# EnVision-Research/Uni-Renderer

Measured on AMD Instinct MI355X. Metric: denoise-steps/sec (dual-UNet, 512^2 bs=4), higher is better.
Workload: dtype f16; 1 GPU; inverse-rendering denoise step: AttributeEncoderModel + UNet2DConditionModel + AttributeDecoderModel forward (SD-1.x size, 1.74 G params, random init), 512x512 image = 64x64 latent, 28-channel attribute latent, 77x768 prompt embedding, batch 4 per GPU; per_gpu_batch=4, global_batch=4, parallelism=dp1, residual_stream=(hi, lo) pairs (parity <= 1e-3, DESIGN.md section 5)

## Files before the change

### include/ur_kernels.h

```cpp
#ifndef UR_KERNELS_H
#define UR_KERNELS_H

#include <stdint.h>

#ifdef __cplusplus
extern "C" {
#endif

#define UR_ABI_VERSION 13

#define UR_E_BADARG (-1001)
#define UR_E_UNSUPPORTED (-1002)

#define UR_DT_F16 0
#define UR_DT_BF16 1
#define UR_DT_F32 2

#define UR_ACT_NONE 0
#define UR_ACT_SILU 1
#define UR_ACT_GEGLU 2

#define UR_TILE_AUTO 0
#define UR_TILE_128x128 1
#define UR_TILE_128x64 2
#define UR_TILE_64x64 3
#define UR_TILE_128x128_S3 4
#define UR_TILE_128x64_S2 5
#define UR_TILE_64x64_S4 6
#define UR_TILE_64x64_S2 7
#define UR_TILE_256x128 8
#define UR_TILE_128x320 9
#define UR_TILE_128x256 10
#define UR_TILE_256x256 11
#define UR_TILE_64x64_R 12
#define UR_TILE_128x64_R 13
#define UR_TILE_128x128_R 14
#define UR_TILE_128x320_R 15
#define UR_TILE_256x128_R 16
#define UR_TILE_64x64_W1 17
#define UR_TILE_128x64_W2 18
#define UR_TILE_64x64_W1_S3 19
#define UR_TILE_64x128_W2 20
// ... 59 lines not shown
    int32_t c0, c1;
    int32_t B, Hin, Win, Hout, Wout;
    int32_t taps, stride, ups;
    int32_t M, N, K;
    int32_t n_store;
    int32_t ld_rowadd, rows_per_b;
    int32_t act;
    float out_scale;
    int32_t zbatch, splitk;
    int32_t zx_div;
    int32_t tile;
    int32_t dtype;
    const void* res_lo;
    void* out_lo;
    int32_t cblock;
    const void* t0;
    const void* t1;
    int64_t ldt0, ldt1, zt0, zt1;
    int32_t ct0, ct1;
    int32_t pad;
    void* out_vt;
    int64_t ldvt, vt_bstride, zvt;
    int32_t vt_n0, vt_rows;
    int32_t zero_page_bytes;
} ur_igemm_desc;

int ur_igemm(const ur_igemm_desc* d, void* stream);

int ur_igemm_uses_dxs(const ur_igemm_desc* d);

int ur_igemm_splitk_gn(const ur_igemm_desc* d, const float* gamma, const float* beta, int64_t zgn, float eps, int groups,
                       int silu, void* stream);

int ur_has_wsconv(void);
int ur_has_pp(void);

int64_t ur_igemm_partial_floats(const ur_igemm_desc* d);

int ur_groupnorm_stats(const void* x0, const void* x1, const void* x0_lo, const void* x1_lo, int c0, int c1, int B,
                       int rows, int groups, int nchunks, float* partial, int dtype, void* stream);
int ur_groupnorm_apply(const void* x0, const void* x1, const void* x0_lo, const void* x1_lo, int c0, int c1, int B,
                       int rows, int groups, int nstat, int nchunks, const float* partial, const float* gamma,
                       const float* beta, float eps, int silu, int bper, int pstride, void* out, int dtype,
                       void* stream);

#define UR_GN_TWO_SWEEP 2
int ur_groupnorm_fused(const void* x0, const void* x1, const void* x0_lo, const void* x1_lo, int c0, int c1, int B,
                       int rows, int groups, const float* gamma, const float* beta, float eps, int silu, int bper,
                       int pstride, void* out, int dtype, void* stream);

int ur_layernorm(const void* x, const void* x_lo, const float* gamma, const float* beta, float eps, int rows, int C,
                 int rows_per_set, int pstride, void* out, int dtype, void* stream);

typedef struct ur_attn_desc {
    const void* q;
    const void* k;
    const void* vt;
    void* o;
    const void* zero_page;
    int64_t ldq, ldk, ldvt, ldo;
    int64_t vt_bstride;
    int64_t q_hstride, k_hstride;
    int32_t q_off, k_off;
    int32_t B, H, Tq, Tk, d;
    float scale;
    int32_t dtype;
// ... 229 lines not shown
```

### uni_renderer_amd/_experiments.py

```python
from __future__ import annotations

import os

KNOWN = {
    "tchain": "row-local chain kernels at the 320-channel level (fused.py)",
    "qkv_one_launch": "q | k | v as one GEMM with a transposed value output (fused.py)",
    "ctxkv_one_launch": "prompt K | V^T of a phase as one GEMM (fused.py)",
    "vt_first": "V^T projection issued before the q | k projection (only without qkv_one_launch)",
    "exchange_early": "exchange GEMMs right behind the kernel that produced their skip (fused.py)",
    "ctx3_early": "up-phase time / prompt projections issued before phase 1 (fused.py)",
    "fold_shortcut": "resnet conv_shortcut as the 1x1 K tail of conv2 (ops.py)",
    "multi_transpose": "batched weight transposes of the backward (backward.py)",
    "batch_wt": "all W^T of a network in one launch group (backward.py)",
    "fused_gradnorm": "clipping norm collected where the gradients are written (backward.py)",
    "wgrad": "weight gradients on ur_wgrad instead of transposed-operand GEMMs (backward.py)",
    "wgrad_table": "measured (tile, slices) table of ur_wgrad (backward.py)",
    "wgrad_defer": "weight gradients deferred to the end of a network's backward and grouped (backward.py)",
    "norm_defer": "gamma / beta gradient sums deferred to the same barriers (backward.py)",
    "heads_multi": "split / merge heads of several tensors in one launch (backward.py)",
    "flash_backward": "flash attention backward instead of the materialised-P path (backward.py)",
    "forward_lse": "the forward attention hands its row log-sum-exp to the backward (backward.py)",
    "batch_casts": "fp32 -> bf16 parameter casts of a network in one launch group (train_step.py)",
    "gn_resident": "one-launch GroupNorm keeps small strips in registers: one memory round trip (ops.py, csrc/norm.hip)",
    "head_major_qk": "the chain kernels write q / k of the d = 40 attention as [sample][head][token][40] images (fused.py)",
    "splitk_gn": "GroupNorm as the split-K second pass (0.07 ms slower: profiles/r04_splitk_gn_ab.txt)",
    "colsum_one_launch": "column sums with an in-launch ticket instead of two launches (slower)",
    "fused_colsum": "bias gradient sums inside the dx GEMM launch (slower)",
    "side_stream": "=1|2|3: independent launches on a sibling graph branch (0.5 ms slower: DESIGN.md)",
    "wsconv": "weight-streaming conv kernel where K >= wsconv_min_k (needs `make WSCONV=1`; slower in the step)",
    "wsconv_min_k": "", "wsconv_waves": "", "zero_page_bytes": "", "conv_cblock": "", "gn_stat_kb": "", "gn_apply_kb": "",
    "gn_apply_max": "", "gn_fused_max_rows": "", "gn_bwd_fused_max_rows": "", "wgrad_tile": "", "wgrad_splits": "",
    "flash_direct_min_d": "", "tchain_min_rows": "", "gn_resident_max_rows": "",
}

RETIRED = {
    "UR_ATTN_BWD_TRN", "UR_BATCH_CASTS", "UR_BATCH_WT", "UR_COLSUM_ONE_LAUNCH", "UR_CONV_CBLOCK", "UR_CTX3_EARLY",
    "UR_CTXKV_ONE_LAUNCH", "UR_EXCHANGE_EARLY", "UR_FLASH_BACKWARD", "UR_FLASH_DIRECT_MIN_D", "UR_FLASH_M32", "UR_FOLD_SHORTCUT",
    "UR_FORWARD_LSE", "UR_FUSED_COLSUM", "UR_FUSED_GRADNORM", "UR_GNF_XCD", "UR_GN_APPLY_KB", "UR_GN_APPLY_MAX",
    "UR_GN_BWD_FUSED_MAX_ROWS", "UR_GN_FUSED_MAX_ROWS", "UR_GN_STAT_KB", "UR_HEADS_MULTI", "UR_MULTI_TRANSPOSE", "UR_NORM_DEFER",
    "UR_NORM_XCD", "UR_QKV_ONE_LAUNCH", "UR_SIDE_STREAM", "UR_SPLITK_GN", "UR_TCHAIN", "UR_TCHAIN_FF", "UR_TCHAIN_PRE",
    "UR_TCHAIN_Q", "UR_TRANSPOSE_MAX", "UR_VT_FIRST", "UR_WGRAD", "UR_WGRAD_DEFER", "UR_WGRAD_SPLITS", "UR_WGRAD_TABLE",
    "UR_WGRAD_TILE", "UR_WSCONV", "UR_WSCONV_MIN_K", "UR_WSCONV_WAVES", "UR_ZERO_PAGE_BYTES",
}

_parsed = None


def _load():
    global _parsed
    if _parsed is None:
        stale = sorted(k for k in os.environ if k in RETIRED)
        if stale:
            raise ValueError(f"retired environment variable(s) {', '.join(stale)}: no longer read -- use UR_EXPERIMENT=... "
                             f"(uni_renderer_amd/_experiments.py lists the entries)")
        d = {}
        for item in os.environ.get("UR_EXPERIMENT", "").replace(";", ",").split(","):
            item = item.strip()
# ... 23 lines not shown
```

### uni_renderer_amd/_lib.py

```python
from __future__ import annotations

import ctypes as C
import os

import torch

_HERE = os.path.dirname(os.path.abspath(__file__))
LIB_PATH = os.environ.get("UR_LIB_PATH", os.path.join(_HERE, "liburhip.so"))
ABI_VERSION = 13

i32, i64, f32, vp = C.c_int32, C.c_int64, C.c_float, C.c_void_p


class IGemmDesc(C.Structure):

    _fields_ = [
        ("x0", vp), ("x1", vp), ("w", vp), ("bias", vp), ("rowadd", vp), ("res", vp), ("out", vp),
        ("partial", vp), ("zero_page", vp),
        ("ldx0", i64), ("ldx1", i64), ("ldw", i64), ("ldres", i64), ("ldc", i64),
        ("zx", i64), ("zw", i64), ("zout", i64), ("zx1", i64), ("zbias", i64), ("zrow", i64), ("zres", i64),
        ("ldp", i64),
        ("c0", i32), ("c1", i32),
        ("B", i32), ("Hin", i32), ("Win", i32), ("Hout", i32), ("Wout", i32),
        ("taps", i32), ("stride", i32), ("ups", i32),
        ("M", i32), ("N", i32), ("K", i32),
        ("n_store", i32), ("ld_rowadd", i32), ("rows_per_b", i32),
        ("act", i32), ("out_scale", f32),
        ("zbatch", i32), ("splitk", i32), ("zx_div", i32), ("tile", i32), ("dtype", i32),
        ("res_lo", vp), ("out_lo", vp),
        ("cblock", i32),
        ("t0", vp), ("t1", vp), ("ldt0", i64), ("ldt1", i64), ("zt0", i64), ("zt1", i64), ("ct0", i32), ("ct1", i32),
        ("pad", i32),
        ("out_vt", vp), ("ldvt", i64), ("vt_bstride", i64), ("zvt", i64), ("vt_n0", i32), ("vt_rows", i32),
        ("zero_page_bytes", i32),
    ]


class AttnDesc(C.Structure):

    _fields_ = [
        ("q", vp), ("k", vp), ("vt", vp), ("o", vp), ("zero_page", vp),
        ("ldq", i64), ("ldk", i64), ("ldvt", i64), ("ldo", i64), ("vt_bstride", i64),
# ... 3 lines not shown
        ("scale", f32), ("dtype", i32),
        ("lse", vp),
    ]


class AttnBwdDesc(C.Structure):

    _fields_ = [
        ("q", vp), ("k", vp), ("v", vp), ("o", vp), ("dout", vp), ("qt", vp), ("kt", vp), ("dot", vp),
        ("ldq", i64), ("ldk", i64), ("ldv", i64), ("ldo", i64), ("lddo", i64), ("ldqt", i64), ("ldkt", i64), ("lddot", i64),
        ("stats", vp), ("dq", vp), ("dk", vp), ("dv", vp),
        ("lddq", i64), ("lddk", i64), ("lddv", i64),
        ("part", vp),
        ("B", i32), ("H", i32), ("d", i32), ("Tq", i32), ("Tk", i32), ("Tk_rows", i32), ("has_lse", i32),
        ("scale", f32), ("dtype", i32),
    ]


class TChainDesc(C.Structure):

    _fields_ = [
        ("a0", vp), ("res", vp), ("res_lo", vp), ("blk", vp), ("blk_lo", vp), ("y_out", vp), ("y_out_lo", vp),
        ("out", vp), ("out_lo", vp), ("out2", vp), ("out3", vp), ("wstream", vp), ("consts", vp),
        ("z_wstream", i64), ("z_consts", i64),
        ("M", i32), ("zbatch", i32), ("mode", i32), ("dtype", i32), ("channels", i32),
        ("rows_per_b", i32), ("ld_vt", i32), ("qk_heads", i32),
        ("eps", f32),
        ("profile", vp),
    ]


SYMBOLS = {
    "ur_igemm": (C.c_int, [C.POINTER(IGemmDesc), vp]),
    "ur_igemm_partial_floats": (C.c_int64, [C.POINTER(IGemmDesc)]),
    "ur_groupnorm_stats": (C.c_int, [vp, vp, vp, vp, C.c_int, C.c_int, C.c_int, C.c_int, C.c_int, C.c_int, vp, C.c_int, vp]),
    "ur_groupnorm_apply": (C.c_int, [vp, vp, vp, vp, C.c_int, C.c_int, C.c_int, C.c_int, C.c_int, C.c_int, C.c_int, vp, vp,
                                     vp, C.c_float, C.c_int, C.c_int, C.c_int, vp, C.c_int, vp]),
    "ur_groupnorm_fused": (C.c_int, [vp, vp, vp, vp, C.c_int, C.c_int, C.c_int, C.c_int, C.c_int, vp, vp, C.c_float,
                                     C.c_int, C.c_int, C.c_int, vp, C.c_int, vp]),
    "ur_layernorm": (C.c_int, [vp, vp, vp, vp, C.c_float, C.c_int, C.c_int, C.c_int, C.c_int, vp, C.c_int, vp]),
    "ur_attention": (C.c_int, [C.POINTER(AttnDesc), vp]),
    "ur_add": (C.c_int, [vp, vp, C.c_float, vp, C.c_int64, C.c_int, vp]),
    "ur_add_hilo": (C.c_int, [vp, vp, vp, vp, C.c_float, vp, vp, C.c_int64, C.c_int, vp]),
    "ur_add_hilo_multi": (C.c_int, [vp, C.c_int, C.c_int, vp]),
    "ur_sizeof_add_item": (C.c_int, []),
    "ur_timestep_embedding": (C.c_int, [vp, C.c_int, C.c_int, C.c_int, C.c_int, C.c_float, vp, C.c_int, vp]),
    "ur_resize_nearest": (C.c_int, [vp, vp, C.c_int, C.c_int, C.c_int, C.c_int, C.c_int, C.c_int, C.c_int, vp]),
    "ur_nchw_to_nhwc": (C.c_int, [vp, C.c_int, C.c_int, C.c_int, C.c_int, C.c_int, vp, C.c_int, C.c_int, vp]),
    "ur_nhwc_to_nchw": (C.c_int, [vp, C.c_int, C.c_int, C.c_int, C.c_int, C.c_int, vp, C.c_int, vp]),
    "ur_ddim_update": (C.c_int, [vp, C.c_int, C.c_int, vp, C.c_int64, C.c_int, C.c_int, C.c_int, vp, vp, C.c_int, vp,
                                 C.c_int, C.c_int, C.c_float, C.c_int, C.c_int, vp]),
    "ur_sampler_advance": (C.c_int, [vp, vp, C.c_int, vp, C.c_int, vp]),
    "ur_select_step_rows": (C.c_int, [vp, vp, vp, C.c_int, vp, C.c_int, vp]),
    "ur_prefetch": (C.c_int, [vp, C.c_int64, C.c_int, vp]),
    "ur_pack_conv_weight": (C.c_int, [vp, vp, C.c_int, C.c_int, C.c_int, C.c_int, vp]),
    "ur_unpack_conv_weight_grad": (C.c_int, [vp, C.c_int64, vp, C.c_int, C.c_int, C.c_int, C.c_int, vp]),
    "ur_unpack_conv_weight_grad_blocks": (C.c_int, [C.c_int, C.c_int]),
    "ur_unpack_conv_weight_grad_sumsq": (C.c_int, [vp, C.c_int64, vp, C.c_int, C.c_int, C.c_int, vp, C.c_int, vp]),
    "ur_unipc_update": (C.c_int, [vp, C.c_int, C.c_int, vp, C.c_int64, C.c_int, C.c_int, C.c_int, vp, vp, C.c_int, vp, vp,
                                  vp, C.c_int, C.c_int, C.c_float, C.c_int, C.c_int, vp]),
    "ur_transpose2d": (C.c_int, [vp, C.c_int64, C.c_int64, vp, C.c_int64, C.c_int64, C.c_int, C.c_int, C.c_int, C.c_int, vp]),
    "ur_im2col3x3_t": (C.c_int, [vp, C.c_int, C.c_int, C.c_int, C.c_int, C.c_int, vp, C.c_int64, C.c_int, vp]),
    "ur_colsum_workspace_floats": (C.c_int64, [C.c_int, C.c_int, C.c_int]),
    "ur_colsum": (C.c_int, [vp, C.c_int64, C.c_int, C.c_int, C.c_int, vp, vp, C.c_int, vp]),
    "ur_colsum_counters": (C.c_int, [C.c_int, C.c_int, C.c_int]),
    "ur_colsum_fused": (C.c_int, [vp, C.c_int64, C.c_int, C.c_int, C.c_int, vp, vp, vp, C.c_int, vp]),
# ... 115 lines not shown
```

### uni_renderer_amd/csrc/igemm.hip

```cpp
#include <cstdlib>

#include "igemm_epi.h"

namespace ur {

template <typename T, int BM, int BN, int WM, int WN, int NSTAGE, bool CONV, int MF, int NL>
__global__ void __launch_bounds__((WM * WN + NL) * 64) igemm_kernel(const ur_igemm_desc p) {
    typedef typename Vec8<T>::type vec8;
    constexpr int NWC = WM * WN;
    constexpr int NW = NL > 0 ? NL : NWC;
    static_assert(NL == 0 || NSTAGE > 0, "loader waves use the LDS-DMA ring");
    constexpr int MREP = BM / WM / 16;
    constexpr int NREP = BN / WN / 16;
    static_assert(MF == 16 || MF == 32, "MFMA shape");
    static_assert(MF == 32 || NREP == 4, "a wave spans 64 output columns (epilogue layout)");
    static_assert(MF == 16 || ((BM / WM) % 32 == 0 && (BN / WN) % 32 == 0), "32x32 MFMA: wave tile in multiples of 32");
    constexpr int MI = BM / WM / 32, NI = BN / WN / 32;
    constexpr int XT_BYTES = BM * 128;
    constexpr int WT_BYTES = BN * 128;
    constexpr int STAGE = XT_BYTES + WT_BYTES;
    constexpr bool REGSTAGE = NSTAGE < 0;
    constexpr int XI = (BM / 8 + NW - 1) / NW;
    constexpr int WI = (BN / 8 + NW - 1) / NW;
    static_assert(NSTAGE <= 2 || ((BM / 8) % NW == 0 && (BN / 8) % NW == 0), "counted vmcnt needs uniform loads per wave");
// ... 706 lines not shown
        case UR_TILE_256x256_M32: return launch_cfg<T, 256, 256, 4, 4, 2, 32>(d, s, reduce);
        case UR_TILE_256x128_M32: return launch_cfg<T, 256, 128, 4, 2, 2, 32>(d, s, reduce);
        case UR_TILE_128x256_M32: return launch_cfg<T, 128, 256, 2, 4, 2, 32>(d, s, reduce);
        case UR_TILE_128x320_L2: return launch_cfg<T, 128, 320, 2, 5, 2, 16, 2>(d, s, reduce);
        case UR_TILE_128x320_L4: return launch_cfg<T, 128, 320, 2, 5, 2, 16, 4>(d, s, reduce);
        case UR_TILE_128x128_L2: return launch_cfg<T, 128, 128, 2, 2, 2, 16, 2>(d, s, reduce);
        case UR_TILE_128x128_S3_L2: return launch_cfg<T, 128, 128, 2, 2, 3, 16, 2>(d, s, reduce);
        case UR_TILE_128x64_L1: return launch_cfg<T, 128, 64, 4, 1, 2, 16, 1>(d, s, reduce);
        case UR_TILE_128x64_S3_L2: return launch_cfg<T, 128, 64, 4, 1, 3, 16, 2>(d, s, reduce);
        case UR_TILE_64x64_S3_L1: return launch_cfg<T, 64, 64, 4, 1, 3, 16, 1>(d, s, reduce);
        case UR_TILE_256x128_L2: return launch_cfg<T, 256, 128, 4, 2, 2, 16, 2>(d, s, reduce);
        case UR_TILE_256x256_L0: return UR_E_UNSUPPORTED;
        case UR_TILE_128x256_L2: return launch_cfg<T, 128, 256, 2, 4, 2, 16, 2>(d, s, reduce);
        case UR_TILE_128x256_S3: return launch_cfg<T, 128, 256, 2, 4, 3>(d, s, reduce);
        case UR_TILE_128x320_W8_M32: return launch_cfg<T, 128, 320, 4, 2, 2, 32>(d, s, reduce);
        case UR_TILE_256x320_W16_M32: return launch_cfg<T, 256, 320, 8, 2, 2, 32>(d, s, reduce);
        case UR_TILE_128x160_M32: return launch_cfg<T, 128, 160, 4, 1, 2, 32>(d, s, reduce);
        case UR_TILE_128x160_S3_M32: return launch_cfg<T, 128, 160, 4, 1, 3, 32>(d, s, reduce);
        case UR_TILE_64x320_M32: return launch_cfg<T, 64, 320, 2, 2, 2, 32>(d, s, reduce);
        case UR_TILE_256x160_W4_M32: return launch_cfg<T, 256, 160, 4, 1, 2, 32>(d, s, reduce);
        case UR_TILE_256x320_W8_M32: return launch_cfg<T, 256, 320, 4, 2, 2, 32>(d, s, reduce);
        case UR_TILE_128x320_W4_M32: return launch_cfg<T, 128, 320, 2, 2, 2, 32>(d, s, reduce);
        case UR_TILE_256x128_W4_M32: return launch_cfg<T, 256, 128, 4, 1, 2, 32>(d, s, reduce);
        case UR_TILE_256x256_W8_M32: return launch_cfg<T, 256, 256, 4, 2, 2, 32>(d, s, reduce);
        case UR_TILE_256x320_W10: return launch_cfg<T, 256, 320, 2, 5, 2>(d, s, reduce);
        case UR_TILE_WS320: return launch_ws<T>(d, s, reduce);
        case UR_TILE_WS320_W8: return launch_ws<T>(d, s, reduce);
        case UR_TILE_PP_128x320: case UR_TILE_PP_128x320_S4: case UR_TILE_PP_256x128: case UR_TILE_PP_128x256:
        case UR_TILE_PP_256x256: case UR_TILE_PP_128x128: case UR_TILE_PP_256x320: return launch_pp<T>(d, s, reduce);
    }
    return UR_E_BADARG;
}

static int64_t padded_ldp(const ur_igemm_desc& d, int tile) {
    const int bn = kTiles[tile].bn;
    return (int64_t)((d.N + bn - 1) / bn) * bn;
}

}

extern "C" int ur_has_pp(void) {
#ifdef UR_WITH_PP
    return 1;
#else
    return 0;
#endif
}

extern "C" int ur_has_wsconv(void) {
#ifdef UR_WITH_WSCONV
    return 1;
#else
    return 0;
#endif
}

extern "C" int64_t ur_igemm_partial_floats(const ur_igemm_desc* d) {
    if (!d || d->splitk <= 1) return 0;
    int64_t ldp = 0;
    for (int t = 1; t < UR_TILE_COUNT; ++t) {
        const int64_t bn = ur::kTiles[t].bn;
        const int64_t v = (d->N + bn - 1) / bn * bn;
        if (v > ldp) ldp = v;
    }
    return (int64_t)d->splitk * (d->zbatch > 1 ? d->zbatch : 1) * d->M * ldp;
}
// ... 83 lines not shown
```

### uni_renderer_amd/ops.py

```python
from __future__ import annotations

import ctypes as C
import json
import math
import os
from typing import Optional, Tuple

import torch

from . import _experiments as X
from . import _lib
from ._lib import AttnDesc, IGemmDesc, check

DT = {torch.float16: 0, torch.bfloat16: 1}
DT_ANY = {torch.float16: 0, torch.bfloat16: 1, torch.float32: 2}
ACT_NONE, ACT_SILU, ACT_GEGLU = 0, 1, 2
TILE_AUTO, TILE_128x128, TILE_128x64, TILE_64x64 = 0, 1, 2, 3
TILE_128x128_S3, TILE_128x64_S2, TILE_64x64_S4, TILE_64x64_S2 = 4, 5, 6, 7
_TILES = {TILE_128x128: (128, 128, 1.0, 2), TILE_128x64: (128, 64, 0.85, 3), TILE_64x64: (64, 64, 0.6, 3),
          TILE_128x128_S3: (128, 128, 0.9, 3), TILE_128x64_S2: (128, 64, 0.7, 2), TILE_64x64_S4: (64, 64, 0.6, 4),
          TILE_64x64_S2: (64, 64, 0.5, 2), 8: (256, 128, 1.1, 2), 9: (128, 320, 1.1, 2), 10: (128, 256, 1.1, 2),
          11: (256, 256, 1.2, 2),
          12: (64, 64, 0.6, "r"), 13: (128, 64, 0.85, "r"), 14: (128, 128, 1.0, "r"), 15: (128, 320, 1.1, "r"),
          16: (256, 128, 1.1, "r"),
# ... 133 lines not shown
        best, best_t = (TILE_64x64, 1), float("inf")
        for tile in _PLANNER_TILES:
            bm, bn, eff, _ = _TILES[tile]
            wgs = math.ceil(M / bm) * math.ceil(N / bn) * zbatch
            for sk in (1, 2, 4, 8):
                if sk > 1 and (zbatch > 4 or K // 64 < 8 * sk):
                    continue
                waves = math.ceil(wgs * sk / 256)
                tt = waves * bm * bn * (K / sk) * 2 / (per_cu * eff)
                if sk > 1:
                    tt += M * N * 4 * (sk + 1) / 4e12 + 3e-6
                if tt < best_t:
                    best, best_t = (tile, sk), tt
        t = best
    _plan_cache[key] = t
    return t


DXS_TRACE = None


def dxs_active() -> bool:
    d = IGemmDesc()
    d.taps, d.stride, d.pad, d.tile = 9, 1, 1, 9
    d.Hin = d.Win = d.Hout = d.Wout = 64
    d.M = 64 * 64
    return bool(_lib.load().ur_igemm_uses_dxs(C.byref(d)))


def igemm(*, x0, w, out, M, N, K, c0, c1=0, x1=None, ldx0, ldx1=0, ldw, ldc, taps=1, conv=None, stride=1, ups=0,
          bias=None, rowadd=None, rows_per_b=0, res=None, ldres=0, n_store=0, act=ACT_NONE, out_scale=1.0,
          zbatch=1, zx=0, zw=0, zout=0, zx1=0, zbias=0, zrow=0, zres=0, zx_div=1, tile=None, splitk=None,
          res_lo=None, out_lo=None, cblock=0, t0=None, t1=None, ldt0=0, ldt1=0, zt0=0, zt1=0, ct0=0, ct1=0, pad=1,
          out_vt=None, vt_n0=0, vt_rows=0, zvt=0, gn=None):
    _require_gpu(x0)
    lib = _lib.load()
    if tile is None or splitk is None:
        pt, ps = plan_igemm(_plan_rows if (_plan_rows is not None and taps == 1) else M, N, K, taps, zbatch)
        tile = pt if tile is None else tile
        splitk = ps if splitk is None else splitk
    d = IGemmDesc()
    d.x0, d.w, d.out = x0.data_ptr(), w.data_ptr(), out.data_ptr()
    if x1 is not None:
        d.x1, d.ldx1, d.c1, d.zx1 = x1.data_ptr(), ldx1, c1, zx1
    if bias is not None:
        d.bias, d.zbias = bias.data_ptr(), zbias
    if rowadd is not None:
        d.rowadd, d.ld_rowadd, d.rows_per_b, d.zrow = rowadd.data_ptr(), rowadd.stride(0), rows_per_b, zrow
    if res is not None:
        d.res, d.ldres, d.zres = res.data_ptr(), ldres, zres
        if res_lo is not None:
            d.res_lo = res_lo.data_ptr()
    if out_lo is not None:
        d.out_lo = out_lo.data_ptr()
    if cblock:
        d.cblock = cblock
    if out_vt is not None:
        d.out_vt, d.ldvt, d.vt_bstride, d.zvt = out_vt.data_ptr(), out_vt.stride(-2), out_vt.stride(0), zvt
        d.vt_n0, d.vt_rows = vt_n0, vt_rows
    if t0 is not None or t1 is not None:
        d.t0, d.t1, d.ldt0, d.ldt1, d.zt0, d.zt1, d.ct0, d.ct1 = _ptr(t0), _ptr(t1), ldt0, ldt1, zt0, zt1, ct0, ct1
    d.zero_page = zero_page(x0.device).data_ptr()
    d.zero_page_bytes = ZERO_PAGE_BYTES
    d.ldx0, d.ldw, d.ldc, d.c0 = ldx0, ldw, ldc, c0
    if zbatch > 1 or zx or zw or zout:
        d.zx, d.zw, d.zout = zx, zw, zout
    d.zx_div = zx_div
    if conv is not None:
        d.B, d.Hin, d.Win, d.Hout, d.Wout = conv
    d.taps, d.stride, d.ups, d.pad = taps, stride, ups, pad
    d.M, d.N, d.K = M, N, K
    if n_store:
        d.n_store = n_store
    d.act, d.out_scale = act, out_scale
    d.zbatch, d.splitk, d.tile, d.dtype = zbatch, splitk, tile, DT[x0.dtype]
    part = None
    if splitk > 1:
        part = torch.empty(int(lib.ur_igemm_partial_floats(C.byref(d))), dtype=torch.float32, device=x0.device)
        d.partial = part.data_ptr()
    if bias is not None and bias.dtype != torch.float32:
        raise RuntimeError("bias must be fp32")
    if DXS_TRACE is not None:
        DXS_TRACE.append(int(lib.ur_igemm_uses_dxs(C.byref(d))))
    e0 = _prof_begin()
    if gn is not None:
        if splitk <= 1:
            raise RuntimeError("igemm(gn=...) is the fused second pass of a split-K launch")
        gam, bet, zgn, eps, groups, silu = gn
        check(lib.ur_igemm_splitk_gn(C.byref(d), gam.data_ptr(), bet.data_ptr(), int(zgn), float(eps), int(groups), int(silu),
                                     _stream()), "ur_igemm_splitk_gn")
    else:
        check(lib.ur_igemm(C.byref(d), _stream()), "ur_igemm")
    if e0 is not None:
        el = x0.element_size()
        z = max(zbatch, 1)
        key = (f"igemm_{_TILES[tile][0]}x{_TILES[tile][1]}s{_TILES[tile][3]}_{'conv3x3' if taps == 9 else 'gemm'}"
               + ("_splitk" if splitk > 1 else "") + ("_gn" if gn is not None else ""))
        if _prof_by_shape:
            key += f"|M{M}_N{N}_K{K}_z{z}_sk{splitk}"
        in_rows = M * (stride * stride if taps == 9 else 1) / (4 ** ups if taps == 9 else 1)
        n_out = N / 2 if act == ACT_GEGLU else N
        lo_el = 1 if x0.dtype == torch.float16 else el
        lo_bytes = M * n_out * lo_el * ((res_lo is not None) + (out_lo is not None))
        _prof_end(e0, key, 2.0 * M * N * K * z,
                  ((in_rows * (K - ct0 - ct1) / taps + M * (ct0 + ct1) + N * K + M * n_out * (1 + (res is not None))) * el
                   + lo_bytes) * z)
    return out


PRECISE_RESIDUAL = os.environ.get("UR_PRECISE_RESIDUAL", "1") != "0"


def lo_of(t):
    return getattr(t, "lo", None) if t is not None else None


def view_hilo(t, *shape):
    v = t.view(*shape)
    lo = lo_of(t)
    if lo is not None:
        v.lo = lo.view(*shape)
    return v


def lo_dtype(dtype):
    return torch.uint8 if dtype == torch.float16 else dtype


def lo_float(lo: torch.Tensor) -> torch.Tensor:
    if lo.dtype == torch.uint8:
# ... 21 lines not shown
    M = x.numel() // K0 // streams
    N = w.shape[-2]
    n_out = N // 2 if act == ACT_GEGLU else N
    vt, vkw = None, {}
    if vt_cols:
        if act != ACT_NONE or res is not None or rowadd is not None or vt_tokens <= 0 or vt_tokens % 64 or (M % vt_tokens):
            raise ValueError("linear(vt_cols=...): plain projection of whole samples with a multiple of 64 tokens")
        n_out = N - vt_cols
        vt = torch.empty(streams * (M // vt_tokens), vt_cols, vt_tokens, dtype=x.dtype, device=x.device)
        vkw = dict(out_vt=vt, vt_n0=n_out, vt_rows=vt_tokens, zvt=(M // vt_tokens) * vt_cols * vt_tokens, n_store=n_out)
    if out is None:
        out = torch.empty(*x.shape[:-1], n_out, dtype=x.dtype, device=x.device)
    _with_lo(out, hilo and act != ACT_GEGLU)
    if res_lo is None:
        res_lo = lo_of(res)
    z = {}
    if streams > 1:
        z = dict(zbatch=streams, zx=M * K0, zx1=M * K1, zw=w.stride(0), zout=M * n_out,
                 zbias=(bias.stride(0) if bias is not None else 0),
                 zres=(res_zstride if res_zstride is not None else M * n_out) if res is not None else 0,
                 zrow=(rowadd.stride(0) * (rowadd.shape[0] // streams)) if rowadd is not None else 0)
    igemm(x0=x, x1=x1, w=w, out=out, M=M, N=N, K=K0 + K1, c0=K0, c1=K1, ldx0=K0, ldx1=K1, ldw=w.stride(-2), ldc=n_out,
          bias=bias, res=res, ldres=(n_out if res is not None else 0), act=act, out_scale=out_scale, rowadd=rowadd,
          rows_per_b=rows_per_b, tile=tile, splitk=splitk, res_lo=res_lo, out_lo=lo_of(out), **z, **vkw)
    return out if vt is None else (out, vt)


CONV_CBLOCK = X.number("conv_cblock", 320)
FOLD_SHORTCUT = X.flag("fold_shortcut", True)


def conv_cblock(cin: int) -> int:
    return CONV_CBLOCK if (CONV_CBLOCK > 0 and cin > CONV_CBLOCK and cin % CONV_CBLOCK == 0) else 0


WSCONV = X.flag("wsconv", False)
WS_C = 320


def wsconv_images(w: torch.Tensor, n_out: Optional[int] = None) -> torch.Tensor:
    N = n_out if n_out is not None else w.shape[0]
    K = w.shape[1]
    if N % WS_C or K % WS_C:
        raise RuntimeError("wsconv_images: N and K must be multiples of 320")
    v = w[:N].reshape(N // WS_C, WS_C, K // 64, 8, 8).permute(0, 2, 1, 3, 4)
    r = torch.arange(WS_C, device=w.device)
    pos = torch.arange(8, device=w.device)[None, :] ^ ((r >> 1) & 7)[:, None]
    idx = pos[None, None, :, :, None].expand(v.shape[0], v.shape[1], WS_C, 8, 8)
    return torch.gather(v, 3, idx).reshape(-1).contiguous()


def pp_built() -> bool:
    return bool(_lib.load().ur_has_pp())


def wsconv_built() -> bool:
    return bool(_lib.load().ur_has_wsconv())


def wsconv_ok(x, N, *, x1=None, stride=1, ups=False, pad=1, tail=None, streams=1) -> bool:
    if x1 is not None or stride != 1 or ups or pad != 1:
        return False
    Bt, H, W, C0 = x.shape
    if (H * W) % 128 or N % WS_C or C0 % WS_C or (C0 > WS_C and conv_cblock(C0) != WS_C):
        return False
    if tail is not None and any(t is not None and t.shape[-1] % WS_C for t in tail):
# ... 32 lines not shown
    if ups:
        Ho, Wo = 2 * H, 2 * W
    elif pad == 0:
        if stride != 2:
            raise RuntimeError("conv3x3: pad=0 is the asymmetric (0, 1, 0, 1) padding of the stride-2 VAE downsample")
        Ho, Wo = (H + 1 - 3) // 2 + 1, (W + 1 - 3) // 2 + 1
    else:
        Ho, Wo = (H + 2 - 3) // stride + 1, (W + 2 - 3) // stride + 1
    N = n_out if n_out is not None else w.shape[-2]
    out = _with_lo(torch.empty(Bt, Ho, Wo, N, dtype=x.dtype, device=x.device), hilo)
    M = B * Ho * Wo
    z = {}
    if streams > 1:
        z = dict(zbatch=streams, zx=B * H * W * C0, zx1=B * H * W * C1, zw=w.stride(0), zout=M * N,
                 zbias=(bias.stride(0) if bias is not None else 0), zres=(M * N if res is not None else 0),
                 zrow=(rowadd.stride(0) * B) if rowadd is not None else 0)
    tl = {}
    if tail is not None:
        ta, tb = tail
        ca, cb_ = ta.shape[-1], (tb.shape[-1] if tb is not None else 0)
        tl = dict(t0=ta, t1=tb, ldt0=ca, ldt1=cb_, ct0=ca, ct1=cb_,
                  zt0=(M * ca if streams > 1 else 0), zt1=(M * cb_ if streams > 1 else 0))
    Kt = 9 * (C0 + C1) + sum(tl.get(k, 0) for k in ("ct0", "ct1"))
    ldw = w.stride(-2)
    if ws is not None and tile in (None, TILE_WS320, TILE_WS320_W8) and wsconv_built() and wsconv_ok(x, N, x1=x1, stride=stride, ups=ups, pad=pad, tail=tail, streams=streams):
        if C0 > WS_C and cblock != WS_C:
            raise RuntimeError("conv3x3: the weight-streaming kernel walks K in the cblock = 320 order")
        w, tile, ldw = ws, (WSCONV_TILE if tile is None else tile), 8
        if streams > 1:
            z["zw"] = ws.stride(0)
        if splitk is None:
            splitk = wsconv_splitk(M, N, Kt, streams)
    gkw = {}
    if gn is not None:
        gam, bet, eps, groups, silu = gn
        if tile is None or splitk is None:
            pt, ps = plan_igemm(M, N, Kt, 9, streams)
            tile, splitk = (pt if tile is None else tile), (ps if splitk is None else splitk)
        if SPLITK_GN and splitk > 1 and res is None and not hilo and splitk_gn_ok(Ho * Wo, N, groups) and min(splitk, Kt // 64) > 1:
            gkw = dict(gn=(gam, bet, (gam.stride(0) if streams > 1 else 0), eps, groups, silu))
    igemm(x0=x, x1=x1, w=w, out=out, M=M, N=N, K=Kt, c0=C0, c1=C1, ldx0=C0, ldx1=C1,
          ldw=ldw, ldc=N, taps=9, conv=(B, H, W, Ho, Wo), stride=stride, ups=int(ups), bias=bias,
          rowadd=rowadd, rows_per_b=Ho * Wo, res=res, ldres=(N if res is not None else 0), out_scale=out_scale,
          tile=tile, splitk=splitk, res_lo=lo_of(res), out_lo=lo_of(out), cblock=cblock, pad=pad, **tl, **z, **gkw)
    if gn is not None and not gkw:
        return groupnorm(out, gam, bet, eps, groups=groups, silu=silu, streams=streams)
    return out


SPLITK_GN = X.flag("splitk_gn", False)


def splitk_gn_ok(rows: int, N: int, groups: int) -> bool:
    return N % groups == 0 and (N // groups) % 4 == 0 and rows * (N // groups) <= 16384


def vt_proj(x, wv, streams=1, shared_x=False):
    Bx, T, Cin = x.shape
    B = Bx if shared_x else Bx // streams
    Cout = wv.shape[-2]
    Tpad = (T + 63) // 64 * 64
    out = torch.empty(streams * B, Cout, Tpad, dtype=x.dtype, device=x.device)
    if shared_x and streams > 1:
        for s_ in range(streams):
            igemm(x0=wv[s_], w=x, out=out[s_ * B:(s_ + 1) * B], M=Cout, N=T, K=Cin, c0=Cin, ldx0=wv.stride(-2), ldw=Cin,
                  ldc=Tpad, n_store=Tpad, zbatch=B, zx=0, zw=T * Cin, zout=Cout * Tpad, splitk=1)
        return out
    igemm(x0=wv, w=x, out=out, M=Cout, N=T, K=Cin, c0=Cin, ldx0=wv.stride(-2), ldw=Cin, ldc=Tpad, n_store=Tpad,
          zbatch=streams * B, zx=(wv.stride(0) if streams > 1 else 0), zx_div=B, zw=T * Cin, zout=Cout * Tpad, splitk=1)
    return out


_GN_STAT_KB = X.number("gn_stat_kb", 64)
_GN_APPLY_KB = X.number("gn_apply_kb", 20)
_GN_APPLY_MAX = X.number("gn_apply_max", 128)


# ... 274 lines not shown
```

Baseline: 85.04 denoise-steps/sec.

## Add LDS-resident-input conv kernel for small-map 3x3 convolutions

Adds a new HIP kernel for 3x3 convs on small feature maps (at most 8x8 spatial, at most 256 rows). It keeps the whole input channel slab in LDS and streams weights through a three-stage ring with direct global-to-LDS loads. Each 160-channel slab writes an fp32 partial, and a separate split-K reduce pass applies the epilogue. The kernel is enabled by default and is meant to cut the weight-bandwidth and occupancy cost of the deep low-resolution UNet convs. In exchange it adds a partial buffer, an extra reduce launch, and a new code path whose correctness has to be kept.

```diff
diff --git a/include/ur_kernels.h b/include/ur_kernels.h
--- a/include/ur_kernels.h
+++ b/include/ur_kernels.h
@@ -7,7 +7,7 @@
 extern "C" {
 #endif
 
-#define UR_ABI_VERSION 13
+#define UR_ABI_VERSION 14
 
 #define UR_E_BADARG (-1001)
 #define UR_E_UNSUPPORTED (-1002)
@@ -133,6 +133,9 @@
 int ur_igemm_splitk_gn(const ur_igemm_desc* d, const float* gamma, const float* beta, int64_t zgn, float eps, int groups,
                        int silu, void* stream);
 
+int ur_conv_resident(const ur_igemm_desc* d, void* stream);
+int ur_conv_resident_slabs(const ur_igemm_desc* d);
+
 int ur_has_wsconv(void);
 int ur_has_pp(void);
 
diff --git a/uni_renderer_amd/_experiments.py b/uni_renderer_amd/_experiments.py
--- a/uni_renderer_amd/_experiments.py
+++ b/uni_renderer_amd/_experiments.py
@@ -23,6 +23,8 @@
     "batch_casts": "fp32 -> bf16 parameter casts of a network in one launch group (train_step.py)",
     "gn_resident": "one-launch GroupNorm keeps small strips in registers: one memory round trip (ops.py, csrc/norm.hip)",
     "head_major_qk": "the chain kernels write q / k of the d = 40 attention as [sample][head][token][40] images (fused.py)",
+    "conv_resident": "small-map 3x3 convs on the LDS-resident-input / streamed-weight kernel (ops.py, csrc/conv_resident.hip)",
+    "conv_resident_nt": "non-temporal weight loads in the small-map conv kernel (profiles/r07_conv_resident_ab.txt)",
     "splitk_gn": "GroupNorm as the split-K second pass (0.07 ms slower: profiles/r04_splitk_gn_ab.txt)",
     "colsum_one_launch": "column sums with an in-launch ticket instead of two launches (slower)",
     "fused_colsum": "bias gradient sums inside the dx GEMM launch (slower)",
diff --git a/uni_renderer_amd/_lib.py b/uni_renderer_amd/_lib.py
--- a/uni_renderer_amd/_lib.py
+++ b/uni_renderer_amd/_lib.py
@@ -7,7 +7,7 @@
 
 _HERE = os.path.dirname(os.path.abspath(__file__))
 LIB_PATH = os.environ.get("UR_LIB_PATH", os.path.join(_HERE, "liburhip.so"))
-ABI_VERSION = 13
+ABI_VERSION = 14
 
 i32, i64, f32, vp = C.c_int32, C.c_int64, C.c_float, C.c_void_p
 
@@ -77,6 +77,8 @@
 
 SYMBOLS = {
     "ur_igemm": (C.c_int, [C.POINTER(IGemmDesc), vp]),
+    "ur_conv_resident": (C.c_int, [C.POINTER(IGemmDesc), vp]),
+    "ur_conv_resident_slabs": (C.c_int, [C.POINTER(IGemmDesc)]),
     "ur_igemm_partial_floats": (C.c_int64, [C.POINTER(IGemmDesc)]),
     "ur_groupnorm_stats": (C.c_int, [vp, vp, vp, vp, C.c_int, C.c_int, C.c_int, C.c_int, C.c_int, C.c_int, vp, C.c_int, vp]),
     "ur_groupnorm_apply": (C.c_int, [vp, vp, vp, vp, C.c_int, C.c_int, C.c_int, C.c_int, C.c_int, C.c_int, C.c_int, vp, vp,
diff --git a/uni_renderer_amd/csrc/conv_resident.hip b/uni_renderer_amd/csrc/conv_resident.hip
--- /dev/null
+++ b/uni_renderer_amd/csrc/conv_resident.hip
@@ -0,0 +1,288 @@
+#include "igemm_epi.h"
+
+namespace ur {
+
+int igemm_reduce_launch(const ur_igemm_desc& d, hipStream_t s);
+
+constexpr int CR_CB = 160;
+constexpr int CR_BN = 80;
+constexpr int CR_ROWS = 256;
+constexpr int CR_KS = CR_CB / 32;
+constexpr int CR_NF = CR_BN / 16;
+constexpr int CR_PIECES = CR_KS * CR_NF;
+constexpr int CR_NW = 8;
+constexpr int CR_MF = CR_ROWS / CR_NW / 16;
+constexpr int CR_NST = 3;
+constexpr int CR_ROW_BYTES = CR_CB * 2;
+constexpr int CR_IMG_BYTES = (CR_ROWS + 1) * CR_ROW_BYTES;
+constexpr int CR_STAGE_BYTES = CR_PIECES * 1024;
+constexpr int CR_LDS = CR_IMG_BYTES + CR_NST * CR_STAGE_BYTES;
+static_assert(CR_LDS <= 160 * 1024, "image + weight ring must fit the 160 KB of a CU");
+
+struct CrPlan { int nb0, nb1, nbt0, nbt1; };
+
+template <typename T, int AUX>
+__global__ void __launch_bounds__(CR_NW * 64) conv_resident_kernel(const ur_igemm_desc p, const CrPlan pl) {
+    typedef typename Vec8<T>::type vec8;
+    extern __shared__ __attribute__((aligned(16))) char smem[];
+    char* img = smem;
+    char* ring = smem + CR_IMG_BYTES;
+
+    const int tid = threadIdx.x, lane = tid & 63;
+    const int wave = __builtin_amdgcn_readfirstlane(tid >> 6);
+    const int l15 = lane & 15, q = lane >> 4;
+
+    const int tiles_n = (p.N + CR_BN - 1) / CR_BN;
+    const int UM = pl.nb0 + pl.nb1, UT = pl.nbt0 + pl.nbt1;
+    const int lid = xcd_remap(blockIdx.x, gridDim.x);
+    const int tile_n = lid % tiles_n;
+    const int u = (lid / tiles_n) % UM;
+    const int zb = lid / (tiles_n * UM);
+    const int n0 = tile_n * CR_BN;
+
+    const int pc0 = p.c0, pc1 = p.c1, pct0 = p.ct0, pct1 = p.ct1, cblk = p.cblock;
+    const T* x0 = reinterpret_cast<const T*>(p.x0) + (int64_t)(zb / p.zx_div) * p.zx;
+    const T* x1 = reinterpret_cast<const T*>(p.x1) + (int64_t)zb * p.zx1;
+    const T* t0 = reinterpret_cast<const T*>(p.t0) + (int64_t)zb * p.zt0;
+    const T* t1 = reinterpret_cast<const T*>(p.t1) + (int64_t)zb * p.zt1;
+    const char* wp = reinterpret_cast<const char*>(reinterpret_cast<const T*>(p.w) + (int64_t)zb * p.zw);
+    const char* zp = reinterpret_cast<const char*>(p.zero_page) + (lane & 7) * 16;
+
+    const int nph = 1 + (UT > u ? (UT - u + UM - 1) / UM : 0);
+    const int S = 9 + (nph - 1);
+
+    const T* ph_src;
+    int64_t ph_ld;
+    int ph_cbeg, ph_nch, ph_kcol0, ph_tapstride;
+    auto set_phase = [&](int ph, const T*& src, int64_t& ld, int& cbeg, int& nch, int& kcol0, int& tapstride) __attribute__((always_inline)) {
+        if (ph == 0) {
+            const bool second = u >= pl.nb0;
+            src = second ? x1 : x0;
+            ld = second ? p.ldx1 : p.ldx0;
+            cbeg = (second ? u - pl.nb0 : u) * CR_CB;
+            nch = min(CR_CB, (second ? pc1 : pc0) - cbeg);
+            if (cblk > 0) {
+                kcol0 = (cbeg / cblk) * 9 * cblk + cbeg % cblk;
+                tapstride = cblk;
+            } else {
+                kcol0 = (second ? pc0 : 0) + cbeg;
+                tapstride = pc0 + pc1;
+            }
+        } else {
+            const int v = u + (ph - 1) * UM;
+            const bool second = v >= pl.nbt0;
+            src = second ? t1 : t0;
+            ld = second ? p.ldt1 : p.ldt0;
+            cbeg = (second ? v - pl.nbt0 : v) * CR_CB;
+            nch = min(CR_CB, (second ? pct1 : pct0) - cbeg);
+            kcol0 = 9 * (pc0 + pc1) + (second ? pct0 : 0) + cbeg;
+            tapstride = 0;
+        }
+    };
+    auto stage_cols = [&](int s, int& kcol, int& nks) __attribute__((always_inline)) {
+        const T* src; int64_t ld; int cbeg, nch, kcol0, tapstride;
+        set_phase(s < 9 ? 0 : s - 8, src, ld, cbeg, nch, kcol0, tapstride);
+        kcol = kcol0 + (s < 9 ? s : 0) * tapstride;
+        nks = nch >> 5;
+    };
+
+    auto swz = [](int row) __attribute__((always_inline)) { return (0x78 >> (2 * ((row >> 2) & 3))) & 3; };
+    constexpr int WI = (CR_PIECES + CR_NW - 1) / CR_NW;
+    static_assert(CR_PIECES % CR_NW == 1, "counted vmcnt: wave 0 issues WI pieces per stage, every other wave WI - 1");
+    const char* wrow[WI];
+    bool wok[WI];
+#pragma unroll
+    for (int i = 0; i < WI; ++i) {
+        const int piece = wave + CR_NW * i;
+        const int ks = piece / CR_NF, nf = piece - ks * CR_NF;
+        const int r = lane >> 2;
+        const int n = n0 + nf * 16 + r;
+        wok[i] = n < p.N;
+        wrow[i] = wp + ((int64_t)n * p.ldw + ks * 32 + ((lane & 3) ^ swz(r)) * 8) * (int64_t)sizeof(T);
+    }
+    int ld_kcol = 0, ld_nks = 0;
+    char* ld_dst = ring;
+    auto issue_begin = [&](int s) __attribute__((always_inline)) {
+        int kcol, nks;
+        stage_cols(s, kcol, nks);
+        ld_kcol = __builtin_amdgcn_readfirstlane(kcol);
+        ld_nks = __builtin_amdgcn_readfirstlane(nks);
+        ld_dst = ring + (s % CR_NST) * CR_STAGE_BYTES;
+    };
+    auto issue_piece = [&](int i) __attribute__((always_inline)) {
+        const int piece = wave + CR_NW * i;
+        if (piece < CR_PIECES) {
+            const int ks = piece / CR_NF;
+            const char* g = (wok[i] && ks < ld_nks) ? wrow[i] + (int64_t)ld_kcol * (int64_t)sizeof(T) : zp;
+            __builtin_amdgcn_global_load_lds((const __attribute__((address_space(1))) void*)g,
+                                             (__attribute__((address_space(3))) void*)(ld_dst + piece * 1024), 16, 0, AUX);
+        }
+    };
+    auto issue = [&](int s) __attribute__((always_inline)) {
+        issue_begin(s);
+#pragma unroll
+        for (int i = 0; i < WI; ++i) issue_piece(i);
+    };
+
+    constexpr int II = CR_ROWS * CR_ROW_BYTES / 1024 / CR_NW;
+    auto stage_image = [&]() __attribute__((always_inline)) {
+        const char* src = reinterpret_cast<const char*>(ph_src);
+#pragma unroll
+        for (int i = 0; i < II; ++i) {
+            const int piece = wave + CR_NW * i;
+            const int g = piece * 64 + lane;
+            const int pix = g / (CR_CB / 8), pos = g - pix * (CR_CB / 8);
+            const int c = (((pos >> 2) << 2) + ((pos & 3) ^ swz(pix))) * 8;
+            const bool ok = pix < p.M && c < ph_nch;
+            glds16(ok ? src + ((int64_t)pix * ph_ld + ph_cbeg + c) * (int64_t)sizeof(T) : zp, img + piece * 1024);
+        }
+    };
+
+    if (tid < CR_ROW_BYTES / 16) *reinterpret_cast<u32x4*>(img + CR_ROWS * CR_ROW_BYTES + tid * 16) = u32x4{0u, 0u, 0u, 0u};
+    __syncthreads();
+    set_phase(0, ph_src, ph_ld, ph_cbeg, ph_nch, ph_kcol0, ph_tapstride);
+    stage_image();
+    issue(0);
+    if (1 < S) issue(1);
+
+    const int hw = p.Hout * p.Wout, Wd = p.Wout, Hd = p.Hout;
+    int pb[CR_MF], py[CR_MF], px[CR_MF];
+#pragma unroll
+    for (int mf = 0; mf < CR_MF; ++mf) {
+        const int m = wave * (16 * CR_MF) + mf * 16 + l15;
+        const int b = m / hw, rem = m - b * hw;
+        py[mf] = (m < p.M) ? rem / Wd : -(1 << 20);
+        px[mf] = rem - (rem / Wd) * Wd;
+        pb[mf] = b * hw;
+    }
+
+    f32x4 acc[CR_MF][CR_NF];
+#pragma unroll
+    for (int mf = 0; mf < CR_MF; ++mf)
+#pragma unroll
+        for (int nf = 0; nf < CR_NF; ++nf) acc[mf][nf] = f32x4{0.f, 0.f, 0.f, 0.f};
+
+    for (int s = 0; s < S; ++s) {
+        if (s + 1 < S) {
+            if (wave == 0) asm volatile("s_waitcnt vmcnt(%0)" ::"n"(WI) : "memory");
+            else asm volatile("s_waitcnt vmcnt(%0)" ::"n"(WI - 1) : "memory");
+        } else {
+            asm volatile("s_waitcnt vmcnt(0)" ::: "memory");
+        }
+        __builtin_amdgcn_s_barrier();
+        asm volatile("" ::: "memory");
+        const bool more = s + 2 < S;
+        if (more) issue_begin(s + 2);
+        if (s >= 9) {
+            set_phase(s - 8, ph_src, ph_ld, ph_cbeg, ph_nch, ph_kcol0, ph_tapstride);
+            stage_image();
+            asm volatile("s_waitcnt vmcnt(0)" ::: "memory");
+            __builtin_amdgcn_s_barrier();
+            asm volatile("" ::: "memory");
+        }
+        const int tap = s < 9 ? s : 4;
+        const int dy = tap / 3 - 1, dx = tap - (tap / 3) * 3 - 1;
+        const char* xrow[CR_MF];
+#pragma unroll
+        for (int mf = 0; mf < CR_MF; ++mf) {
+            const int iy = py[mf] + dy, ix = px[mf] + dx;
+            const bool ok = ((unsigned)iy < (unsigned)Hd) && ((unsigned)ix < (unsigned)Wd);
+            const int row = ok ? pb[mf] + iy * Wd + ix : CR_ROWS;
+            xrow[mf] = img + row * CR_ROW_BYTES + ((q ^ swz(row)) << 4);
+        }
+        const char* ws = ring + (s % CR_NST) * CR_STAGE_BYTES + ((l15 * 4 + (q ^ swz(l15))) << 4);
+#pragma unroll
+        for (int ks = 0; ks < CR_KS; ++ks) {
+            vec8 wf[CR_NF], xf[CR_MF];
+#pragma unroll
+            for (int nf = 0; nf < CR_NF; ++nf) wf[nf] = *reinterpret_cast<const vec8*>(ws + (ks * CR_NF + nf) * 1024);
+#pragma unroll
+            for (int mf = 0; mf < CR_MF; ++mf) xf[mf] = *reinterpret_cast<const vec8*>(xrow[mf] + ks * 64);
+            if (more) {
+                if (ks < WI) issue_piece(ks);
+                if (ks + CR_KS < WI) issue_piece(ks + CR_KS);
+            }
+#pragma unroll
+            for (int mf = 0; mf < CR_MF; ++mf)
+#pragma unroll
+                for (int nf = 0; nf < CR_NF; ++nf) acc[mf][nf] = mfma16(wf[nf], xf[mf], acc[mf][nf]);
+        }
+    }
+
+    float* slab = p.partial + ((int64_t)(zb * UM + u) * p.M) * p.ldp;
+#pragma unroll
+    for (int mf = 0; mf < CR_MF; ++mf) {
+        const int m = wave * (16 * CR_MF) + mf * 16 + l15;
+        if (m < p.M) {
+#pragma unroll
+            for (int nf = 0; nf < CR_NF; ++nf)
+                *reinterpret_cast<float4*>(slab + (int64_t)m * p.ldp + n0 + nf * 16 + q * 4) =
+                    make_float4(acc[mf][nf][0], acc[mf][nf][1], acc[mf][nf][2], acc[mf][nf][3]);
+        }
+    }
+}
+
+static bool cr_plan(const ur_igemm_desc& d, CrPlan& pl) {
+    if (!d.x0 || !d.w || !d.out || !d.zero_page) return false;
+    if (d.taps != 9 || d.stride != 1 || d.ups || d.pad != 1) return false;
+    if (d.dtype != UR_DT_F16 && d.dtype != UR_DT_BF16) return false;
+    if (d.act == UR_ACT_GEGLU || d.out_vt) return false;
+    if (d.B <= 0 || d.Hout <= 0 || d.Wout <= 0 || d.Hin != d.Hout || d.Win != d.Wout) return false;
+    if (d.Hout * d.Wout > 64 || d.M != d.B * d.Hout * d.Wout || d.M > CR_ROWS || d.N <= 0) return false;
+    if (d.c0 <= 0 || (d.c0 % BK) || d.c1 < 0 || (d.c1 % BK) || (d.c1 > 0 && !d.x1)) return false;
+    if (d.ct0 < 0 || d.ct1 < 0 || (d.ct0 == 0 && d.ct1 != 0) || (d.ct0 % BK) || (d.ct1 % BK)) return false;
+    if ((d.ct0 > 0 && !d.t0) || (d.ct1 > 0 && !d.t1)) return false;
+    if (d.K != 9 * (d.c0 + d.c1) + d.ct0 + d.ct1) return false;
+    if ((d.ldx0 % 8) || (d.c1 > 0 && (d.ldx1 % 8)) || (d.ldw % 8) || (d.ct0 > 0 && (d.ldt0 % 8)) || (d.ct1 > 0 && (d.ldt1 % 8))) return false;
+    if (d.cblock < 0 || (d.cblock > 0 && ((d.cblock % CR_CB) || d.c1 != 0 || (d.c0 % d.cblock)))) return false;
+    if (d.rowadd && d.rows_per_b <= 0) return false;
+    if (d.zero_page_bytes != 0 && d.zero_page_bytes < 256) return false;
+    pl.nb0 = (d.c0 + CR_CB - 1) / CR_CB;
+    pl.nb1 = (d.c1 + CR_CB - 1) / CR_CB;
+    pl.nbt0 = (d.ct0 + CR_CB - 1) / CR_CB;
+    pl.nbt1 = (d.ct1 + CR_CB - 1) / CR_CB;
+    return true;
+}
+
+template <typename T, int AUX>
+static void cr_launch(const ur_igemm_desc& d, const CrPlan& pl, dim3 grid, hipStream_t s) {
+    static std::atomic<uint64_t> done{0};
+    set_lds_limit_once(done, reinterpret_cast<const void*>(&conv_resident_kernel<T, AUX>), CR_LDS);
+    hipLaunchKernelGGL((conv_resident_kernel<T, AUX>), grid, dim3(CR_NW * 64), CR_LDS, s, d, pl);
+}
+
+}
+
+extern "C" int ur_conv_resident_slabs(const ur_igemm_desc* d) {
+    ur::CrPlan pl;
+    if (!d || !ur::cr_plan(*d, pl)) return UR_E_BADARG;
+    return pl.nb0 + pl.nb1;
+}
+
+extern "C" int ur_conv_resident(const ur_igemm_desc* din, void* stream) {
+    using namespace ur;
+    CrPlan pl;
+    if (!din || !cr_plan(*din, pl)) return UR_E_BADARG;
+    ur_igemm_desc d = *din;
+    if (d.zbatch < 1) d.zbatch = 1;
+    if (d.zx_div < 1) d.zx_div = 1;
+    const int slabs = pl.nb0 + pl.nb1;
+    if (!d.partial || (d.splitk != 0 && d.splitk != slabs)) return UR_E_BADARG;
+    d.splitk = slabs;
+    if (d.n_store <= 0) d.n_store = d.N;
+    const int tiles_n = (d.N + CR_BN - 1) / CR_BN;
+    d.ldp = (int64_t)tiles_n * CR_BN;
+    hipStream_t s = reinterpret_cast<hipStream_t>(stream);
+    const dim3 grid(tiles_n * slabs * d.zbatch);
+    const bool nt = din->tile == 1;
+    if (d.dtype == UR_DT_F16) {
+        if (nt) cr_launch<f16, 2>(d, pl, grid, s);
+        else cr_launch<f16, 0>(d, pl, grid, s);
+    } else {
+        if (nt) cr_launch<bf16, 2>(d, pl, grid, s);
+        else cr_launch<bf16, 0>(d, pl, grid, s);
+    }
+    const hipError_t e = hipGetLastError();
+    if (e != hipSuccess) return -(int)e;
+    return igemm_reduce_launch(d, s);
+}
diff --git a/uni_renderer_amd/csrc/igemm.hip b/uni_renderer_amd/csrc/igemm.hip
--- a/uni_renderer_amd/csrc/igemm.hip
+++ b/uni_renderer_amd/csrc/igemm.hip
@@ -762,6 +762,22 @@
     return UR_E_BADARG;
 }
 
+int igemm_reduce_launch(const ur_igemm_desc& d, hipStream_t s) {
+    const int64_t total = (int64_t)d.M * (d.ldp / 16);
+    int blocks = (int)((total + 255) / 256);
+    if (blocks > 4096) blocks = 4096;
+    const bool pipe = total * d.zbatch < REDUCE_PIPE_MAX_THREADS;
+    if (d.dtype == UR_DT_F16) {
+        if (pipe) hipLaunchKernelGGL((igemm_splitk_reduce<f16, true>), dim3(blocks, d.zbatch), dim3(256), 0, s, d);
+        else hipLaunchKernelGGL((igemm_splitk_reduce<f16, false>), dim3(blocks, d.zbatch), dim3(256), 0, s, d);
+    } else {
+        if (pipe) hipLaunchKernelGGL((igemm_splitk_reduce<bf16, true>), dim3(blocks, d.zbatch), dim3(256), 0, s, d);
+        else hipLaunchKernelGGL((igemm_splitk_reduce<bf16, false>), dim3(blocks, d.zbatch), dim3(256), 0, s, d);
+    }
+    const hipError_t e = hipGetLastError();
+    return e == hipSuccess ? 0 : -(int)e;
+}
+
 static int64_t padded_ldp(const ur_igemm_desc& d, int tile) {
     const int bn = kTiles[tile].bn;
     return (int64_t)((d.N + bn - 1) / bn) * bn;
diff --git a/uni_renderer_amd/ops.py b/uni_renderer_amd/ops.py
--- a/uni_renderer_amd/ops.py
+++ b/uni_renderer_amd/ops.py
@@ -189,10 +189,12 @@
           bias=None, rowadd=None, rows_per_b=0, res=None, ldres=0, n_store=0, act=ACT_NONE, out_scale=1.0,
           zbatch=1, zx=0, zw=0, zout=0, zx1=0, zbias=0, zrow=0, zres=0, zx_div=1, tile=None, splitk=None,
           res_lo=None, out_lo=None, cblock=0, t0=None, t1=None, ldt0=0, ldt1=0, zt0=0, zt1=0, ct0=0, ct1=0, pad=1,
-          out_vt=None, vt_n0=0, vt_rows=0, zvt=0, gn=None):
+          out_vt=None, vt_n0=0, vt_rows=0, zvt=0, gn=None, resident=0):
     _require_gpu(x0)
     lib = _lib.load()
-    if tile is None or splitk is None:
+    if resident:
+        tile, splitk = CONV_RESIDENT_NT, resident
+    elif tile is None or splitk is None:
         pt, ps = plan_igemm(_plan_rows if (_plan_rows is not None and taps == 1) else M, N, K, taps, zbatch)
         tile = pt if tile is None else tile
         splitk = ps if splitk is None else splitk
@@ -232,8 +234,9 @@
     d.act, d.out_scale = act, out_scale
     d.zbatch, d.splitk, d.tile, d.dtype = zbatch, splitk, tile, DT[x0.dtype]
     part = None
-    if splitk > 1:
-        part = torch.empty(int(lib.ur_igemm_partial_floats(C.byref(d))), dtype=torch.float32, device=x0.device)
+    if splitk > 1 or resident:
+        floats = int(lib.ur_igemm_partial_floats(C.byref(d))) if splitk > 1 else max(zbatch, 1) * M * (-(-N // 320) * 320)
+        part = torch.empty(floats, dtype=torch.float32, device=x0.device)
         d.partial = part.data_ptr()
     if bias is not None and bias.dtype != torch.float32:
         raise RuntimeError("bias must be fp32")
@@ -246,13 +249,18 @@
         gam, bet, zgn, eps, groups, silu = gn
         check(lib.ur_igemm_splitk_gn(C.byref(d), gam.data_ptr(), bet.data_ptr(), int(zgn), float(eps), int(groups), int(silu),
                                      _stream()), "ur_igemm_splitk_gn")
+    elif resident:
+        check(lib.ur_conv_resident(C.byref(d), _stream()), "ur_conv_resident")
     else:
         check(lib.ur_igemm(C.byref(d), _stream()), "ur_igemm")
     if e0 is not None:
         el = x0.element_size()
         z = max(zbatch, 1)
-        key = (f"igemm_{_TILES[tile][0]}x{_TILES[tile][1]}s{_TILES[tile][3]}_{'conv3x3' if taps == 9 else 'gemm'}"
-               + ("_splitk" if splitk > 1 else "") + ("_gn" if gn is not None else ""))
+        if resident:
+            key = "conv_resident_conv3x3_splitk"
+        else:
+            key = (f"igemm_{_TILES[tile][0]}x{_TILES[tile][1]}s{_TILES[tile][3]}_{'conv3x3' if taps == 9 else 'gemm'}"
+                   + ("_splitk" if splitk > 1 else "") + ("_gn" if gn is not None else ""))
         if _prof_by_shape:
             key += f"|M{M}_N{N}_K{K}_z{z}_sk{splitk}"
         in_rows = M * (stride * stride if taps == 9 else 1) / (4 ** ups if taps == 9 else 1)
@@ -340,6 +348,21 @@
 
 def conv_cblock(cin: int) -> int:
     return CONV_CBLOCK if (CONV_CBLOCK > 0 and cin > CONV_CBLOCK and cin % CONV_CBLOCK == 0) else 0
+
+
+CONV_RESIDENT = X.flag("conv_resident", True)
+CONV_RESIDENT_CB = 160
+CONV_RESIDENT_NT = int(X.flag("conv_resident_nt", False))
+
+
+def conv_resident_slabs(H, W, rows, C0, C1=0, *, stride=1, ups=False, pad=1, cblock=0, tail=None) -> int:
+    if stride != 1 or ups or pad != 1 or H * W > 64 or rows > 256:
+        return 0
+    if C0 % 64 or C1 % 64 or (cblock and (cblock % CONV_RESIDENT_CB or C1 or C0 % cblock)):
+        return 0
+    if tail is not None and any(t is not None and t.shape[-1] % 64 for t in tail):
+        return 0
+    return -(-C0 // CONV_RESIDENT_CB) + -(-C1 // CONV_RESIDENT_CB)
 
 
 WSCONV = X.flag("wsconv", False)
@@ -438,9 +461,14 @@
         if splitk is None:
             splitk = wsconv_splitk(M, N, Kt, streams)
     gkw = {}
+    rkw = {}
+    if CONV_RESIDENT and ws is None and tile is None and splitk is None and not (gn is not None and SPLITK_GN):
+        slabs = conv_resident_slabs(H, W, M, C0, C1, stride=stride, ups=ups, pad=pad, cblock=cblock, tail=tail)
+        if slabs:
+            rkw = dict(resident=slabs)
     if gn is not None:
         gam, bet, eps, groups, silu = gn
-        if tile is None or splitk is None:
+        if not rkw and (tile is None or splitk is None):
             pt, ps = plan_igemm(M, N, Kt, 9, streams)
             tile, splitk = (pt if tile is None else tile), (ps if splitk is None else splitk)
         if SPLITK_GN and splitk > 1 and res is None and not hilo and splitk_gn_ok(Ho * Wo, N, groups) and min(splitk, Kt // 64) > 1:
@@ -448,7 +476,7 @@
     igemm(x0=x, x1=x1, w=w, out=out, M=M, N=N, K=Kt, c0=C0, c1=C1, ldx0=C0, ldx1=C1,
           ldw=ldw, ldc=N, taps=9, conv=(B, H, W, Ho, Wo), stride=stride, ups=int(ups), bias=bias,
           rowadd=rowadd, rows_per_b=Ho * Wo, res=res, ldres=(N if res is not None else 0), out_scale=out_scale,
-          tile=tile, splitk=splitk, res_lo=lo_of(res), out_lo=lo_of(out), cblock=cblock, pad=pad, **tl, **z, **gkw)
+          tile=tile, splitk=splitk, res_lo=lo_of(res), out_lo=lo_of(out), cblock=cblock, pad=pad, **tl, **z, **gkw, **rkw)
     if gn is not None and not gkw:
         return groupnorm(out, gam, bet, eps, groups=groups, silu=silu, streams=streams)
     return out
```

Result: no change. 85.81 denoise-steps/sec (median of 6 runs) (+0.9%).
